# ryanelandt/PressureFieldContact.jl

Hardware: AMD Instinct MI355X
Metric: tet-tri clip+integrate ops/s (higher is better)
Workload: dtype f64

## Files before the change

pressurefieldcontact.jl_amd/csrc/pfc_hip.hip:

```cpp
#include "pfc_kernels.h"

#include <atomic>
#include <condition_variable>
#include <functional>
#include <mutex>
#include <thread>
#include <cmath>
#include <cstdlib>
#include <limits>
#include <cstdarg>
#include <cstdio>
#include <cstring>
#include <string>
#include <vector>

#include "../../include/pfc.h"
#include "pfc_sort.h"

namespace pfc {

__global__ void k_prep_tri(int n, const double *__restrict__ pt, const int *__restrict__ tri, TriRec *__restrict__ out) {
    int k = blockIdx.x * blockDim.x + threadIdx.x;
    if (k >= n) return;
    V3 a = ld3(pt + 3 * tri[3 * k]), b = ld3(pt + 3 * tri[3 * k + 1]), c = ld3(pt + 3 * tri[3 * k + 2]);
// ... 324 lines not shown
    bool want_surv = false;
    int opt_graph = 1;
    size_t fcap = 0, ccap = 0, tcap = 0, rcap = 0;
    DevBuf<double> h_pose;
    int last_n_items = 0, last_levels = 0, last_bfs_levels = 0;
    bool pending = false;
    hipStream_t last_stream = nullptr;
    long long stats[8] = {0, 0, 0, 0, 0, 0, 0, 0};
    DevBuf<double> dual_in, dual_acc, dual_res, dual_out, dual_poly;
    DevBuf<int2> dual_pkey;
    DevBuf<int> dual_sel, dual_flag;
    DevBuf<double> scat_d;
    DevBuf<int> scat_i;
    DevBuf<double> sdual_d, sdual_w;
    DevBuf<int> sdual_i;
    DevBuf<char> sdual_tmp;
    DevBuf<int> surv;
    DevBuf<int> rgn;
    DevBuf<int> poly_item, pcnt, poly_cand;
    DevBuf<double> poly;
    long long last_undecided = 0;
    long long last_active = 0;
    struct ShapeHint { int n = 0; bool sparse = false; } hints[4];
    void note_shape(int n, bool sparse) {
        int k = 0;
        while (k < 3 && hints[k].n != n) ++k;
        for (; k > 0; --k) hints[k] = hints[k - 1];
        hints[0].n = n; hints[0].sparse = sparse;
    }
    bool shape_is_sparse(int n) const {
        for (const ShapeHint &e : hints) if (e.n == n) return e.sparse;
        return false;
    }
    long long last_tslots = 0;
    Event ev[EV_COUNT];
    bool ev_valid = false;
    pfc_context *twin = nullptr;
    bool is_twin = false;
    DevBuf<int> fout;
    PinBuf<int> h_fout;
    int *fout_dev = nullptr;
    const int *fout_host = nullptr;
    int opt_fused = 1;
    int opt_fixed_order = 0;
    DevBuf<int> det;
    DevBuf<unsigned long long> sort_keys[2];
    DevBuf<int> canon_off, canon_fill, canon_item;
    int sort_tmp_items = 0;
    bool fixed_whole_list = false;
    DevBuf<char> sort_tmp;
    size_t sort_tmp_for = 0;
    int sort_tmp_bits = 0;
    int max_elem1 = 1, max_elem2 = 1;
    DevBuf<double> fx_rec, vfx_rec;
    DevBuf<int> vfx_head;
    DevBuf<int> fx_head;
    long long surv_sorted_serial = -1;
    size_t sort_cover = 0;
    size_t sort_cover_used = 0;
    int opt_vertex_fields = 1;
    int opt_clip_queue = 1;
    int fused_skip = 0;
    int fused_seq = 0;
    int fu_nw = 1;
    int last_fu_nw = 0, last_team = 0;
    int n_cu = 0;
    int opt_team = 48;
    DevBuf<unsigned long long> team;
    DevBuf<int> emit_ctr;
    PinBuf<int> h_emit;
    PinBuf<unsigned> h_more;
    bool fu_emit = false;
    int dual_fused_skip = 0;
    const double *fu_dpose = nullptr, *fu_dtwist = nullptr;
    double *fu_dwrench = nullptr, *fu_dsdot = nullptr;
    int fu_ndir = 0;
    bool pending_fused = false, last_fused = false;
    int opt_split_min = 1025;
    int opt_clip_min = 384;
    int opt_poison = 0;
    int split_n0 = 0;
    bool in_split = false;
    int last_parts = 1;
    Event ev_fork, ev_join, ev_join0;
    int twin_queue_fallback = 0;
    DevBuf<long long> surf_cnt, surf_off, surf_out;
    DevBuf<double> surf_part;
    DevBuf<int> surf_seg, surf_canon_off, surf_canon_fill, surf_canon_item;
    DevBuf<double> ljac_seed;
    DevBuf<double> ljac_out;
    DevBuf<double> ljac_io;
    DevBuf<int> ljac_ids;
    std::vector<int> ins_bodies;
    DevBuf<int> bodies_bind;
    bool bodies_stale = true;
    DevBuf<double> bodies_d;
    DevBuf<int> bodies_i;
    DevBuf<unsigned long long> surf_keys[2];
    DevBuf<char> surf_tmp;
    PinBuf<long long> h_surf;
    bool pending_surface = false;
    bool surf_whole_list = false;
    bool surf_cap_short = false;
    int surf_n_ctr = 0;
    long long surf_cap_poly = 0, surf_cap_trac = 0;
    DevBuf<long long> surf_hl;
// ... 230 lines not shown

int record_eval(pfc_context *h, int n_items, const int *d_ins_ids, const double *d_pose, const double *d_twist,
                const double *d_s, double *d_wrench, double *d_sdot, int *d_counts, hipStream_t st, bool prof) {
    new_value_pass(h);
    h->pending_more = false; h->last_dual_reused = false;
    const int levels = eff_levels(h);
    int *ccount = h->ctr.p, *tcount = h->ctr.p + 1, *next_seed = h->ctr.p + 2;
    int *ucount = h->ctr.p + 4, *fcount = h->ctr.p + 6;
    int *pcount = h->ctr.p + ((levels + 9) & ~1);
#ifdef PFC_STAMPS
    HIP_TRY(h, hipMemsetAsync(h->stamps.p, 0, sizeof(unsigned long long) * 16, st));
#endif
    if (prof) HIP_TRY(h, hipEventRecord(h->ev[EV_START], st));

    EvalArgs ea;
    ea.n_items = n_items; ea.ins_ids = d_ins_ids; ea.pose = d_pose; ea.twist = d_twist; ea.s = d_s;
    ea.bp_pose = h->bp_dev;
    ea.ins = h->d_ins; ea.meshes = h->d_meshes; ea.n_ins = (int)h->ins.size(); ea.items = h->items.p;
    ea.frontier0 = h->frontier[0].p; ea.fcount = fcount; ea.acc = h->acc.p; ea.icnt = h->icnt.p;
    ea.status = h->status.p;
    hipLaunchKernelGGL(k_setup_items, dim3(grid_for(n_items, 64, 1 << 20)), dim3(64), 0, st, ea);
    if (prof) HIP_TRY(h, hipEventRecord(h->ev[EV_SETUP], st));

    const int L = bfs_levels_for(h, n_items, levels);
    launch_broadphase(h, n_items, L, ccount, fcount, next_seed, ucount, st);
    if (h->bp_dev)
        hipLaunchKernelGGL(k_repose, dim3(grid_for(n_items, 64, 1 << 20)), dim3(64), 0, st, n_items, d_pose, h->items.p);
    if (h->opt_fixed_order) {
        int ba, bb;
        const int bits = pfc_sort_key_bits(n_items, h->max_elem1, h->max_elem2, &ba, &bb);
        if (bits > 64)
            return fail(h, PFC_ERR_BAD_ARG, "option fixed_order: (item, element, element) needs %d key bits for %d items, more than 64", bits, n_items);
        size_t cover = h->sort_cover ? h->sort_cover : h->ccap;
        if (cover > h->ccap) cover = h->ccap;
        h->sort_cover_used = cover;
        static const bool global_sort = std::getenv("PFC_FIXED_GLOBAL_SORT") != nullptr;
        if (global_sort || h->fixed_whole_list)
            HIP_TRY(h, pfc_sort_candidates(h->cand.p, ccount, cover, h->sort_keys[0].p, h->sort_keys[1].p, h->sort_tmp.p, h->sort_tmp.cap,
                                           n_items, ba, bb, bits, h->status.p, kStFixedCover, st));
        else
            HIP_TRY(h, pfc_canon_candidates(h->cand.p, ccount, cover, h->icnt.p, n_items, h->sort_keys[0].p, h->sort_keys[1].p, h->canon_off.p,
                                            h->canon_fill.p, h->canon_item.p, bb, h->status.p, kStFixedCover, kStFixedBig, st));
        hipLaunchKernelGGL(k_fixed_init, dim3(grid_for(n_items, 256, 1 << 20)), dim3(256), 0, st, n_items, h->det.p);
    }
    if (prof) HIP_TRY(h, hipEventRecord(h->ev[EV_BP], st));

    NpArgs np;
    np.items = h->items.p; np.cand = h->cand.p; np.ccount = ccount; np.ccap = (int)h->ccap; np.acc = h->acc.p;
    np.icnt = h->icnt.p; np.n_items = n_items; np.clip_n = h->opt_debug ? h->clip_n.p : nullptr; np.trac = trac_view(h);
    np.tcount = tcount; np.tcap = (int)h->tcap; np.status = h->status.p; np.debug = h->opt_debug;
    np.stamps = h->stamps.p;
    np.rec = h->rec.p; np.rgn = h->rgn.p; np.rr_cap = (int)(h->rcap / kRgn);
    np.poly_item = h->poly_item.p; np.poly = h->poly.p; np.pcap = (int)poly_cap(h->ccap);
    np.pcnt = h->pcnt.p; np.chunk_switch = kNpChunkSwitch; np.poly_cand = h->want_surv ? h->poly_cand.p : nullptr;
    np.surv = h->want_surv ? h->surv.p : nullptr; np.scount = pcount + 1;
    const int np_grid = grid_for(h->ccap, kNpBlock, kNpMaxBlocks);
    const int np_mode = h->opt_debug ? 1 : ((h->opt_fixed_order || (h->opt_clip_min > 0 && n_items >= h->opt_clip_min)) ? 2 : 0);
    if (np_mode == 1) {
        if (h->any_tet_tet) hipLaunchKernelGGL((k_narrow<true, 1>), dim3(np_grid), dim3(kNpBlock), 0, st, np);
        else hipLaunchKernelGGL((k_narrow<false, 1>), dim3(np_grid), dim3(kNpBlock), 0, st, np);
    } else if (np_mode == 0) {
        if (h->any_tet_tet) hipLaunchKernelGGL((k_narrow<true, 0>), dim3(np_grid), dim3(kNpBlock), 0, st, np);
        else hipLaunchKernelGGL((k_narrow<false, 0>), dim3(np_grid), dim3(kNpBlock), 0, st, np);
    } else {
        if (h->opt_clip_queue && !h->any_tet_tet) {
            hipLaunchKernelGGL(k_clip_queue, dim3(np_grid), dim3(kNpBlock), 0, st, np);
        } else if (h->in_split || (n_items >= 640 && n_items < 1024)) {
            if (h->any_tet_tet) hipLaunchKernelGGL((k_narrow<true, 3>), dim3(np_grid), dim3(kNpBlock), 0, st, np);
            else hipLaunchKernelGGL((k_narrow<false, 3>), dim3(np_grid), dim3(kNpBlock), 0, st, np);
        } else {
            if (h->any_tet_tet) hipLaunchKernelGGL((k_narrow<true, 2>), dim3(np_grid), dim3(kNpBlock), 0, st, np);
            else hipLaunchKernelGGL((k_narrow<false, 2>), dim3(np_grid), dim3(kNpBlock), 0, st, np);
        }
        IntegArgs ig;
        ig.items = h->items.p; ig.n_items = n_items; ig.ccount = ccount; ig.ccap = (int)h->ccap; ig.chunk_switch = kNpChunkSwitch;
        ig.pcnt = h->pcnt.p; ig.poly_item = h->poly_item.p; ig.poly = h->poly.p; ig.pcap = np.pcap;
        ig.poly_cand = np.poly_cand; ig.surv = np.surv; ig.scount = np.scount; ig.acc = h->acc.p; ig.rec = h->rec.p;
        ig.rgn = h->rgn.p; ig.rr_cap = np.rr_cap; ig.icnt = h->icnt.p; ig.status = h->status.p;
        ig.det = h->opt_fixed_order ? h->det.p : nullptr;
        if (h->opt_fixed_order) hipLaunchKernelGGL(k_integ_fixed, dim3(grid_for(h->ccap, 64, kNpMaxBlocks)), dim3(64), 0, st, ig);
        else hipLaunchKernelGGL(k_integ, dim3(grid_for(h->ccap, 64, kNpMaxBlocks)), dim3(64), 0, st, ig);
    }
    if (prof) HIP_TRY(h, hipEventRecord(h->ev[EV_NP], st));

    BrArgs br;
    br.items = h->items.p; br.n_items = n_items; br.acc = h->acc.p; br.res = h->res.p; br.icnt = h->icnt.p;
    br.trac = trac_view(h); br.tcount = tcount; br.tcap = (int)h->tcap; br.wrench = d_wrench; br.sdot = d_sdot;
    br.counts = d_counts;
    br.ctr = h->ctr.p; br.n_ctr = levels + 12; br.status = h->status.p; br.tail = h->tail_dev ? h->tail_dev : h->tail.p;
    br.rgn = h->rgn.p; br.i_pcount = (levels + 9) & ~1;
    if (h->opt_fixed_order && np_mode == 2) {
        FixedArgs fx;
        fx.rec = h->rec.p; fx.det = h->det.p; fx.n_items = n_items; fx.n_slots = (int)(h->rcap / kRgn) * kRgn; fx.items = h->items.p;
        fx.acc = h->acc.p; fx.status = h->status.p;
        hipLaunchKernelGGL(k_shift_fixed, dim3(n_items), dim3(64), 0, st, fx);
    }
    if (h->any_bristle) {
        ShiftArgs sh;
        sh.rec = h->rec.p; sh.rgn = h->rgn.p; sh.rr_cap = (int)(h->rcap / kRgn); sh.acc = h->acc.p;
        if (!(h->opt_fixed_order && np_mode == 2)) hipLaunchKernelGGL(k_shift, dim3(grid_for(h->rcap, 64, 2048)), dim3(64), 0, st, sh);
        hipLaunchKernelGGL(k_eig, dim3(n_items), dim3(64), 0, st, br);
        FricArgs fr;
        fr.items = h->items.p; fr.poly_item = h->poly_item.p; fr.poly = h->poly.p; fr.ccount = ccount; fr.ccap = (int)h->ccap;
        fr.chunk_switch = kNpChunkSwitch; fr.pcnt = h->pcnt.p;
        fr.pcap = np.pcap; fr.res = h->res.p; fr.acc = h->acc.p;
        fr.n_items = n_items; fr.status = h->status.p;
// ... 740 lines not shown
    }
    h->finalized = true;
    return PFC_OK;
}

static int check_eval_args(pfc_context *h, int n_items, const void *ins_ids, const void *pose, const void *twist,
                           const void *s, const void *wrench, const void *sdot) {
    if (!h->finalized) return fail(h, PFC_ERR_STATE, "pfc_eval before pfc_finalize");
    if (n_items < 0) return fail(h, PFC_ERR_BAD_ARG, "negative n_items");
    if (n_items == 0) return PFC_OK;
    if (h->ins.empty()) return fail(h, PFC_ERR_STATE, "no contact instructions");
    if (!pose || !twist || !wrench || !sdot) return fail(h, PFC_ERR_BAD_ARG, "null buffer");
    if (!ins_ids && n_items > (int)h->ins.size())
        return fail(h, PFC_ERR_BAD_ARG, "n_items exceeds the number of instructions and no ins_ids given");
    if (h->any_bristle && !s) return fail(h, PFC_ERR_BAD_ARG, "bristle instructions need the state buffer s");
    return PFC_OK;
}

int pfc_eval_device(pfc_handle h, int n_items, const int *d_ins_ids, const double *d_pose, const double *d_twist,
                    const double *d_s, double *d_wrench, double *d_sdot, int *d_counts, void *stream) {
    if (!h) return PFC_ERR_BAD_ARG;
    if (h->multi)
        return multi_eval_device(h, n_items, 0, d_ins_ids, d_pose, nullptr, d_twist, d_s, nullptr, nullptr, nullptr, d_wrench, d_sdot,
                                 nullptr, nullptr, d_counts, stream);
    { const int rc = check_eval_args(h, n_items, d_ins_ids, d_pose, d_twist, d_s, d_wrench, d_sdot); if (rc != PFC_OK) return rc; }
    if (n_items == 0) { h->pending = false; h->last_n_items = 0; return PFC_OK; }
    HIP_TRY(h, hipSetDevice(h->device));
    hipStream_t st = stream ? (hipStream_t)stream : h->stream;
    h->split_n0 = 0;
    h->pending_fused = false;
    end_kept_pass(h);
    h->pending_more = false;
    int team = fused_team(h, n_items);
    if (team > 1 && !team_acquire(h)) team = fused_ok(h, n_items) ? 1 : 0;
    if (team) {
        h->fu_nw = team;
        const int rc_t = enqueue_fused(h, n_items, d_ins_ids, d_pose, d_twist, d_s, d_wrench, d_sdot, d_counts, st);
        h->fu_nw = 1;
        if (rc_t != PFC_OK) team_release(h);
        return rc_t;
    }
    if (h->fused_skip > 0 && n_items <= kFusedMaxItems) --h->fused_skip;
    const bool split = h->opt_split_min > 0 && n_items >= h->opt_split_min && d_ins_ids && !h->opt_debug && !h->opt_fixed_order &&
                       !h->want_surv && !h->is_twin && !pile_mode(h, n_items);
    if (!split) return enqueue_eval(h, n_items, d_ins_ids, d_pose, d_twist, d_s, d_wrench, d_sdot, d_counts, st);
    int rc = make_twin(h);
    if (rc != PFC_OK) return rc;
    pfc_context *t = h->twin;
    t->opt_profile = h->opt_profile; t->opt_max_levels = h->opt_max_levels; t->opt_bfs_levels = h->opt_bfs_levels;
    t->opt_poison = h->opt_poison;
    if (t->opt_clip_min != h->opt_clip_min) { t->opt_clip_min = h->opt_clip_min; t->ghave[0] = t->ghave[1] = false; }
    if (t->opt_clip_queue != h->opt_clip_queue) { t->opt_clip_queue = h->opt_clip_queue; t->ghave[0] = t->ghave[1] = false; }
    if (t->opt_vertex_fields != h->opt_vertex_fields) { t->opt_vertex_fields = h->opt_vertex_fields; t->ghave[0] = t->ghave[1] = false; }
    t->opt_graph = h->opt_graph;
    if (t->opt_no_filter != h->opt_no_filter) { t->opt_no_filter = h->opt_no_filter; t->ghave[0] = t->ghave[1] = false; }
    const int n0 = n_items / 2, n1 = n_items - n0;
    hipStream_t s0 = h->stream;
    HIP_TRY(h, hipEventRecord(h->ev_fork, st));
    if (s0 != st) HIP_TRY(h, hipStreamWaitEvent(s0, h->ev_fork, 0));
    HIP_TRY(h, hipStreamWaitEvent(t->stream, h->ev_fork, 0));
    h->in_split = true; t->in_split = true;
    rc = enqueue_eval(h, n0, d_ins_ids, d_pose, d_twist, d_s, d_wrench, d_sdot, d_counts, s0);
    h->in_split = false;
    if (rc != PFC_OK) return rc;
    rc = enqueue_eval(t, n1, d_ins_ids + n0, d_pose + 24 * (size_t)n0, d_twist + 6 * (size_t)n0,
                      d_s ? d_s + 6 * (size_t)n0 : nullptr, d_wrench + 6 * (size_t)n0, d_sdot + 6 * (size_t)n0,
                      d_counts ? d_counts + 4 * (size_t)n0 : nullptr, t->stream);
    if (rc != PFC_OK) { h->err = t->err; return rc; }
    HIP_TRY(h, hipEventRecord(h->ev_join, t->stream));
    HIP_TRY(h, hipStreamWaitEvent(st, h->ev_join, 0));
    if (s0 != st) {
        HIP_TRY(h, hipEventRecord(h->ev_join0, s0));
        HIP_TRY(h, hipStreamWaitEvent(st, h->ev_join0, 0));
    }
    h->split_n0 = n0;
    return PFC_OK;
}

namespace {

struct SurfFricOut {
    const double *s;
    double *fric, *fric_summary, *stiff;
};

int surface_enqueue(pfc_context *h, int n_items, const int *d_ins_ids, const double *d_pose, const double *d_twist, long long cap_poly,
                    long long cap_trac, long long *d_poly_off, int *d_poly_idx, double *d_poly_xyz, long long *d_poly_trac,
                    double *d_trac, double *d_summary, int *d_counts, long long *d_totals, hipStream_t st, const SurfFricOut *fo = nullptr) {
    new_value_pass(h);
    h->pending_more = false;
    h->pin_in_pt = {}; h->pin_din_pt = {};
    h->pending = false; h->pending_dual = false; h->pending_dual_hyb = false; h->split_n0 = 0;
    if (h->pending_fused) { h->pending_fused = false; team_release(h); }
    int ba, bb;
    const int bits = pfc_sort_key_bits(n_items, h->max_elem1, h->max_elem2, &ba, &bb);
    if (bits > 64)
        return fail(h, PFC_ERR_BAD_ARG, "pfc_contact_surface: (item, element, element) needs %d key bits for %d items, more than 64", bits, n_items);
    HIP_TRY(h, ensure_work(h, n_items));
    const size_t c = h->ccap;
    HIP_TRY(h, h->surf_cnt.ensure(2 * (c + 1)));
    HIP_TRY(h, h->surf_off.ensure(2 * (c + 1)));
    HIP_TRY(h, h->surf_part.ensure(c * kSurfSums));
    HIP_TRY(h, h->surf_seg.ensure((size_t)n_items + 1));
    HIP_TRY(h, h->surf_canon_off.ensure((size_t)n_items + 1));
    HIP_TRY(h, h->surf_canon_fill.ensure((size_t)n_items));
    HIP_TRY(h, h->surf_canon_item.ensure(c));
// ... 1315 lines not shown
    }
    h->want_surv = true;
    int rc = pfc_eval(h, n_items, ins_ids, pose, twist, s, wrench, sdot, counts);
    h->want_surv = false;
    if (rc != PFC_OK) return rc;
    HIP_TRY(h, ensure_graphed(h, h->dual_in, nk * 36));
    HIP_TRY(h, ensure_graphed(h, h->dual_acc, nk * kDaStride));
    HIP_TRY(h, ensure_graphed(h, h->dual_res, nk * kDrStride));
    HIP_TRY(h, ensure_graphed(h, h->dual_out, nk * 12));
    double *dp = h->dual_in.p, *dt = dp + nk * 24, *dsd = dt + nk * 6;
    const size_t in_bytes = sizeof(double) * nk * 36, out_bytes = sizeof(double) * nk * 12;
    HIP_TRY(h, h->pin_in.ensure(in_bytes));
    HIP_TRY(h, h->pin_out.ensure(out_bytes));
    pack_seeds((double *)h->pin_in.p, nk, d_pose, d_twist, d_s, true);
    HIP_TRY(h, hipMemcpyAsync(dp, h->pin_in.p, in_bytes, hipMemcpyHostToDevice, st));
    rc = launch_dual(h, n_items, n_dir, h->tail.p, dp, dt, dsd, h->dual_out.p, h->dual_out.p + nk * 6, (size_t)h->stats[2], st, nullptr);
    if (rc != PFC_OK) return rc;
    h->dual_hint = h->stats[2];
    HIP_TRY(h, hipMemcpyAsync(h->pin_out.p, h->dual_out.p, out_bytes, hipMemcpyDeviceToHost, st));
    HIP_TRY(h, hipStreamSynchronize(st));
    copy_out_dual((const double *)h->pin_out.p, nk, d_wrench, d_sdot);
    return PFC_OK;
}

int pfc_set_option(pfc_handle h, const char *name, long long value) {
    if (!h || !name) return PFC_ERR_BAD_ARG;
    if (h->multi) {
        if (!std::strcmp(name, "multi_min")) { h->multi->opt_min_items = value < 1 ? 1 : (int)value; h->multi->part_n = 0; return PFC_OK; }
        h->multi->dev_kept = false;
        for (pfc_context *c : h->multi->shard) {
            const int rc = on_shard(h, c, [&](pfc_context *c1) { return pfc_set_option(c1, name, value); });
            if (rc != PFC_OK) return rc;
        }
        return PFC_OK;
    }
    end_kept_pass(h);
    if (!std::strcmp(name, "debug")) h->opt_debug = value != 0;
    else if (!std::strcmp(name, "profile")) h->opt_profile = value != 0;
    else if (!std::strcmp(name, "max_levels")) {
        if (value < 0 || value > (1 << 20) || (h->finalized && value > h->max_levels))
            return fail(h, PFC_ERR_BAD_ARG, "max_levels must be 0 (automatic) or 1..%d (depth of the finalized trees + 1)", h->max_levels);
        h->opt_max_levels = (int)value; h->ghave[0] = h->ghave[1] = false; h->dghave = false;
    }
    else if (!std::strcmp(name, "bfs_levels")) h->opt_bfs_levels = (int)value;
    else if (!std::strcmp(name, "graph")) h->opt_graph = value != 0;
    else if (!std::strcmp(name, "split_min")) h->opt_split_min = (int)value;
    else if (!std::strcmp(name, "dual_reuse")) h->opt_dual_reuse = (int)value;
    else if (!std::strcmp(name, "clip_min")) { h->opt_clip_min = (int)value; h->ghave[0] = h->ghave[1] = false; h->dghave = false; }
    else if (!std::strcmp(name, "clip_queue")) { h->opt_clip_queue = (int)value; h->ghave[0] = h->ghave[1] = false; h->dghave = false; }
    else if (!std::strcmp(name, "vertex_fields")) {
        if (value != 0 && value != 1) return fail(h, PFC_ERR_BAD_ARG, "vertex_fields must be 0 (per-point k_fric) or 1 (per-corner fields)");
        h->opt_vertex_fields = (int)value; h->ghave[0] = h->ghave[1] = false; h->dghave = false;
    }
    else if (!std::strcmp(name, "poison")) h->opt_poison = value != 0;
    else if (!std::strcmp(name, "fused")) { h->opt_fused = value != 0; h->fused_skip = 0; }
    else if (!std::strcmp(name, "team")) h->opt_team = value < 0 ? 0 : (value > kTeamMaxWg ? kTeamMaxWg : (int)value);
    else if (!std::strcmp(name, "team_fault")) h->opt_team_fault = (int)value;
    else if (!std::strcmp(name, "fused_f32")) h->opt_fused_f32 = value != 0;
    else if (!std::strcmp(name, "dual_fold")) { h->opt_dual_fold = value != 0; h->dghave = false; }
    else if (!std::strcmp(name, "fixed_order")) {
        const int on = value != 0;
        if (on != h->opt_fixed_order) {
            h->opt_fixed_order = on; h->fused_skip = 0;
            h->ghave[0] = h->ghave[1] = false; h->dghave = false;
            h->rec.release();
        }
    }
    else if (!std::strcmp(name, "no_filter")) { h->opt_no_filter = (int)value; h->ghave[0] = h->ghave[1] = false; h->dghave = false; }
    else return fail(h, PFC_ERR_BAD_ARG, "unknown option %s", name);
    return PFC_OK;
}

int pfc_get_stats(pfc_handle h, long long *out8) {
    if (!h || !out8) return PFC_ERR_BAD_ARG;
    if (h->multi) { for (int k = 0; k < 8; ++k) out8[k] = h->multi->stats[k]; return PFC_OK; }
    for (int k = 0; k < 8; ++k) out8[k] = h->stats[k];
    return PFC_OK;
}

int pfc_get_stage_ms(pfc_handle h, float *out6) {
    if (!h || !out6) return PFC_ERR_BAD_ARG;
    if (h->multi)
        return on_first_shard(h, [&](pfc_context *c) { return pfc_get_stage_ms(c, out6); });
    if (!h->ev_valid) return fail(h, PFC_ERR_STATE, "profile option was off for the last evaluation");
    HIP_TRY(h, hipSetDevice(h->device));
    HIP_TRY(h, hipEventSynchronize(h->ev[EV_FIN]));
    for (int k = 0; k < 5; ++k) HIP_TRY(h, hipEventElapsedTime(&out6[k], h->ev[k], h->ev[k + 1]));
    HIP_TRY(h, hipEventElapsedTime(&out6[5], h->ev[EV_START], h->ev[EV_FIN]));
    if (h->last_parts == 2 && h->twin && h->twin->ev_valid) {
        pfc_context *t = h->twin;
        float b[6];
        HIP_TRY(h, hipEventSynchronize(t->ev[EV_FIN]));
        for (int k = 0; k < 5; ++k) HIP_TRY(h, hipEventElapsedTime(&b[k], t->ev[k], t->ev[k + 1]));
        HIP_TRY(h, hipEventElapsedTime(&b[5], t->ev[EV_START], t->ev[EV_FIN]));
        for (int k = 0; k < 5; ++k) out6[k] = 0.5f * (out6[k] + b[k]);
        if (b[5] > out6[5]) out6[5] = b[5];
    }
    return PFC_OK;
}

int pfc_last_parts(pfc_handle h) { return h ? (h->multi ? pfc_last_parts(h->multi->shard[0]) : (h->last_fused ? 0 : h->last_parts)) : 0; }
int pfc_last_team(pfc_handle h) { return h ? (h->multi ? pfc_last_team(h->multi->shard[0]) : (h->last_fused ? h->last_fu_nw : 0)) : 0; }
int pfc_last_dual_reused(pfc_handle h) {
    if (!h) return 0;
    if (h->multi) {
        for (int k = 0; k < h->multi->n_used; ++k)
// ... 330 lines not shown
```

pressurefieldcontact.jl_amd/csrc/pfc_np.h:

```cpp
#pragma once

struct TracSoA {
    int *item;
    double *nx, *ny, *nz, *rx, *ry, *rz, *dA, *p;
};

struct NpArgs {
    const ItemRec *items;
    const WorkRec *cand;
    const int *ccount;
    int ccap;
    double *acc;
    double *rec;
    int *rgn;
    int rr_cap;
    int *pcnt;
    int chunk_switch;
    int *poly_cand;
    int *icnt;
    int n_items;
    int *clip_n;
    int *poly_item;
    double *poly;
    int pcap;
    int *surv;
    int *scount;
    TracSoA trac;
    int *tcount;
    int tcap;
    unsigned *status;
    int debug;
    unsigned long long *stamps;
};

__device__ __forceinline__ V3 cross_fma(V3 a, V3 b) {
    return V3{__builtin_fma(a.y, b.z, -(a.z * b.y)), __builtin_fma(a.z, b.x, -(a.x * b.z)), __builtin_fma(a.x, b.y, -(a.y * b.x))};
}
__device__ __forceinline__ double dot_fma(V3 a, V3 b) { return __builtin_fma(a.z, b.z, __builtin_fma(a.y, b.y, a.x * b.x)); }
__device__ __forceinline__ V3 axpy_fma(double a, V3 x, V3 y) {
    return V3{__builtin_fma(a, x.x, y.x), __builtin_fma(a, x.y, y.y), __builtin_fma(a, x.z, y.z)};
}

#ifndef PFC_EXP
#define PFC_EXP 0
#endif
constexpr int kElim = PFC_EXP;
constexpr int kNpBlock = 64;
constexpr int kNpChunkBig = 512;
__device__ __forceinline__ int np_chunk(int n_c, int chunk_switch) {
    int C = kNpChunkBig;
    while (C > kNpBlock && (long long)C * chunk_switch > n_c) C >>= 1;
    return C;
}

constexpr int kRingColsClip = 48;
#define PR(k, c) poly[((((rbase) + (k)) & 7) * 4 + (c)) * RC + rcol]

__device__ __forceinline__ double readlane_f64(double v, int src) {
    return __hiloint2double(__builtin_amdgcn_readlane(__double2hiint(v), src),
                            __builtin_amdgcn_readlane(__double2loint(v), src));
}

__device__ __forceinline__ double wave_total(double v, int lane) {
    double t;
    t = dpp_move<0x111, 0xF>(v); v += t;
    t = dpp_move<0x112, 0xF>(v); v += t;
    t = dpp_move<0x114, 0xF>(v); v += t;
    t = dpp_move<0x118, 0xF>(v); v += t;
    t = dpp_move<0x142, 0xA>(v); v += (lane & 16) ? t : 0.0;
    t = dpp_move<0x143, 0xC>(v); v += (lane >= 32) ? t : 0.0;
// ... 657 lines not shown
                const int n_run = __popcll(heads);
                if (lane < n_run && !((rec_done >> lane) & 1ull) && rbase + lane < g.rr_cap)
                    g.rec[(size_t)(rslot0 + rbase + lane) * kRecStride + 1] = 0.0;
            }
            STAMP(r3);
#ifdef PFC_STAMPS
            st_r[0] += r1 - t4; st_r[1] += r2 - r1; st_r[2] += r3 - r2;
#endif
            if (single) {
                const int n_ne = __popcll(__ballot(has_poly));
                const int ntl = contributed ? n_trac_lane : 0;
                int nt = 0;
#pragma unroll
                for (int b = 0; b < 5; ++b) nt += __popcll(__ballot((ntl >> b) & 1)) << b;
                if (lane == 0 && am) {
                    if (n_ne) atomicAdd(&g.icnt[4 * (size_t)item_first + 2], n_ne);
                    if (nt) atomicAdd(&g.icnt[4 * (size_t)item_first + 3], nt);
                }
            } else {
                count_per_item(g.icnt, cw.item, 2, active, has_poly);
                count_per_item(g.icnt, cw.item, 3, active, contributed, n_trac_lane);
            }
        }
#ifdef PFC_STAMPS
        STAMP(t5);
        {
            if (t1 == 0) t1 = t2;
            st_c[0] += t1 - t0; st_c[1] += t2 - t1; st_c[2] += t3 - t2; st_c[3] += t4 - t3; st_c[4] += t5 - t4; st_c[5] += 1;
        }
#endif
    }
    if (lane == 0) g.pcnt[ch] = pc;
    }
#ifdef PFC_STAMPS
    if (lane == 0 && g.stamps && st_c[5])
    {
        for (int k = 0; k < 6; ++k) atomicAdd(&g.stamps[k], st_c[k]);
        atomicAdd(&g.stamps[6], st_r[0]); atomicAdd(&g.stamps[7], st_r[1]); atomicAdd(&g.stamps[14], st_r[2]);
    }
#endif
}
#undef PR

__global__ void __launch_bounds__(kNpBlock) k_clip_queue(NpArgs g) {
    constexpr int RC = kNpBlock;
    __shared__ double poly[8 * 4 * RC];
    __shared__ unsigned short qpos[2 * kNpBlock];
    const int lane = threadIdx.x;
    int n_c = *g.ccount;
    if (n_c > g.ccap) n_c = g.ccap;
    const int C = np_chunk(n_c, g.chunk_switch);
    const int n_chunk = (n_c + C - 1) / C;
    const unsigned long long below = (1ull << lane) - 1ull;
#define QZ(e, k, i) poly[(((((e) >> 6) * 3 + (k)) * 4 + (i)) * RC) + ((e) & 63)]
#define QX(e, i) poly[(((6 + ((e) >> 6)) * 4 + (i)) * RC) + ((e) & 63)]
    for (int ch = blockIdx.x; ch < n_chunk; ch += gridDim.x) {
        const int n_here = n_c - ch * C < C ? n_c - ch * C : C;
        const int n_round = (n_here + kNpBlock - 1) / kNpBlock;
        int q = 0;
        int pc = 0;
        auto dense_round = [&]() {
            const int n_take = q < kNpBlock ? q : kNpBlock;
            const bool mine = lane < n_take, left = kNpBlock + lane < q;
            V3 nh = mk3(0.0, 0.0, 0.0);
            unsigned long long meta = 0ull;
            int pos = 0;
            if (mine) {
                nh = mk3(QX(lane, 0), QX(lane, 1), QX(lane, 2));
                meta = (unsigned long long)__double_as_longlong(QX(lane, 3));
                pos = (int)qpos[lane];
            }
            double zl[3][4], xl[4];
            int posl = 0;
            if (left) {
#pragma unroll
                for (int k = 0; k < 3; ++k)
#pragma unroll
                    for (int i = 0; i < 4; ++i) zl[k][i] = QZ(kNpBlock + lane, k, i);
#pragma unroll
                for (int i = 0; i < 4; ++i) xl[i] = QX(kNpBlock + lane, i);
                posl = (int)qpos[kNpBlock + lane];
            }
            const int item = (int)(unsigned)(meta & 0xFFFFFFFFull), b = (int)(unsigned)(meta >> 32);
            const ItemRec *it = g.items + item;
            const GTetRec *tp = (const GTetRec *)(it->tet + b);
            RingCol<RC> ring{poly, lane, 0};
            int n_poly = 0;
            double V[12] = {0.0, 0.0, 0.0, 0.0, 0.0, 0.0, 0.0, 0.0, 0.0, 0.0, 0.0, 0.0}, E[4] = {0.0, 0.0, 0.0, 0.0};
            if (mine) {
#pragma unroll
                for (int k = 0; k < 12; ++k) V[k] = tp->xrz[k];
#pragma unroll
                for (int k = 0; k < 4; ++k) E[k] = tp->epsr[k];
            }
            if (mine) {
                bool err = false;
                n_poly = clip_ring_in_tet_coordinates(ring, 3, err);
                if (err) atomicOr(g.status, kStNonFinite);
            }
            const bool has_poly = n_poly >= 3;
            const unsigned long long km = __ballot(has_poly);
            const int slot = ch * C + pc + __popcll(km & below);
            pc += __popcll(km);
            if (has_poly) np_keep_polygon(ring, n_poly, V, E, nh, g, slot, item, ch * C + pos);
            if (km) {
                const int item_first = __builtin_amdgcn_readfirstlane(item);
                if (__all(!mine || item == item_first)) {
                    if (lane == 0) atomicAdd(&g.icnt[4 * (size_t)item_first + 2], __popcll(km));
                } else {
                    count_per_item(g.icnt, item, 2, mine, has_poly);
                }
            }
            if (left) {
#pragma unroll
                for (int k = 0; k < 3; ++k)
#pragma unroll
                    for (int i = 0; i < 4; ++i) QZ(lane, k, i) = zl[k][i];
#pragma unroll
                for (int i = 0; i < 4; ++i) QX(lane, i) = xl[i];
                qpos[lane] = (unsigned short)posl;
            }
            q -= n_take;
            wave_lds_sync();
        };
        for (int rd = 0; rd < n_round; ++rd) {
            const int pos = rd * kNpBlock + lane, idx = ch * C + pos;
            bool active = pos < n_here;
            WorkRec cw;
            cw.item = 0; cw.a = 0; cw.b = 0; cw.pad = 0;
            if (active) cw = g.cand[idx];
            if ((unsigned)cw.item >= (unsigned)g.n_items) {
                atomicOr(g.status, kStHole);
                cw.item = 0; cw.a = 0; cw.b = 0;
                active = false;
            }
            const ItemRec *it = g.items + cw.item;
            const GTetRec *tp = (const GTetRec *)(it->tet + cw.b);
            double z[4][4];
            int n_in = 0;
            V3 nh_in = mk3(0.0, 0.0, 0.0);
            bool survivor = false;
            if (active) survivor = np_front<false>(it, cw, tp, z, n_in, nh_in, g.status, true);
            const unsigned long long sm = __ballot(survivor);
            if (survivor) {
                const int e = q + __popcll(sm & below);
#pragma unroll
                for (int k = 0; k < 3; ++k)
#pragma unroll
                    for (int i = 0; i < 4; ++i) QZ(e, k, i) = z[k][i];
                QX(e, 0) = nh_in.x; QX(e, 1) = nh_in.y; QX(e, 2) = nh_in.z;
                QX(e, 3) = __longlong_as_double((long long)(((unsigned long long)(unsigned)cw.b << 32) | (unsigned long long)(unsigned)cw.item));
                qpos[e] = (unsigned short)pos;
            }
            q += __popcll(sm);
            wave_lds_sync();
            if (q >= kNpBlock) dense_round();
        }
        if (q > 0) dense_round();
        if (lane == 0) g.pcnt[ch] = pc;
    }
#undef QZ
#undef QX
}

struct IntegArgs {
    const ItemRec *items;
    int n_items;
    const int *ccount;
    int ccap, chunk_switch;
    const int *pcnt;
    int *poly_item;
    const double *poly;
    int pcap;
    const int *poly_cand;
    int *surv, *scount;
    double *acc, *rec;
    int *rgn;
    int rr_cap;
    int *icnt;
    unsigned *status;
    int *det;
};

template <int N, int L>
__device__ __forceinline__ double lds_rows_total(const double *buf, int lane, int lane0) {
    constexpr int RS = 64 + L;
    static_assert(N * L <= 64 && (L == 1 || L == 2 || L == 4), "rows x lanes per row must fit the wave");
    double t = 0.0;
    const int row = lane / L, part = lane % L;
    if (row < N) {
        const double *r = buf + row * RS + part;
        double t0 = 0.0, t1 = 0.0, t2 = 0.0, t3 = 0.0;
#pragma unroll
        for (int j = 0; j < 64 / L; j += 8) {
            const double a0 = r[L * j], a1 = r[L * (j + 1)], a2 = r[L * (j + 2)], a3 = r[L * (j + 3)];
            const double a4 = r[L * (j + 4)], a5 = r[L * (j + 5)], a6 = r[L * (j + 6)], a7 = r[L * (j + 7)];
            t0 += a0; t1 += a1; t2 += a2; t3 += a3;
            t0 += a4; t1 += a5; t2 += a6; t3 += a7;
        }
        t = (t0 + t1) + (t2 + t3);
    }
#pragma unroll
    for (int m = 1; m < L; m <<= 1) t += __shfl_xor(t, m, 64);
    const int dst_row = lane - lane0;
    const double out = __shfl(t, (dst_row >= 0 && dst_row < N) ? dst_row * L : 0, 64);
    return (dst_row >= 0 && dst_row < N) ? out : 0.0;
}

template <bool DET>
__device__ __forceinline__ void integ_body(const IntegArgs &g, double *m27) {
    constexpr int RS = 66;
    const int lane = threadIdx.x;
    int n_c = *g.ccount;
    if (n_c > g.ccap) n_c = g.ccap;
    const int C = np_chunk(n_c, g.chunk_switch);
    const int n_chunk = (n_c + C - 1) / C;
    const size_t P = (size_t)g.pcap;
    for (int ch = blockIdx.x; ch < n_chunk; ch += gridDim.x) {
        int cnt = __builtin_amdgcn_readfirstlane(g.pcnt[ch]);
        if (cnt > C) cnt = C;
        int cur = -1, n_tr = 0;
        bool cur_reg = false;
        V3 c0 = mk3(0.0, 0.0, 0.0);
        double s10[10];
#pragma unroll
        for (int k = 0; k < 10; ++k) s10[k] = 0.0;
        auto flush = [&]() {
            if (cur < 0 || !__any(n_tr > 0)) return;
            double t10 = 0.0, Wt = 0.0, sx = 0.0, sy = 0.0, sz = 0.0;
#pragma unroll
            for (int k = 0; k < 10; ++k) {
                const double t = wave_total(s10[k], lane);
                if (lane == (DET ? kRecTen + k : k)) t10 = t;
                if (k == 6) Wt = t;
                if (k == 7) sx = t;
                if (k == 8) sy = t;
                if (k == 9) sz = t;
            }
            if constexpr (DET) {
                const bool mom = !cur_reg && Wt > 0.0;
                double mine = 0.0;
                if (mom) {
                    wave_lds_sync();
                    mine = lds_rows_total<27, 2>(m27, lane, 5);
                    if (lane == 1) mine = Wt;
                    if (lane == 2) mine = c0.x;
                    if (lane == 3) mine = c0.y;
                    if (lane == 4) mine = c0.z;
                    if (lane == 32) mine = sx - Wt * c0.x;
                    if (lane == 33) mine = sy - Wt * c0.y;
                    if (lane == 34) mine = sz - Wt * c0.z;
                }
                if (lane == 0) mine = (double)cur;
                if (lane >= kRecTen && lane < kRecTen + 10) mine = t10;
                if (lane == kRecChunk) mine = (double)ch;
                const int rgn_c = ch & (kRgn - 1);
                int rs = 0;
                if (lane == 0) rs = atomicAdd(g.rgn + rgn_c * kRgnStride + 1, 1);
                rs = __builtin_amdgcn_readfirstlane(rs);
                if (rs < g.rr_cap) {
                    const int slot = rgn_c * g.rr_cap + rs;
                    if (lane == kRecNext) mine = (double)atomicExch(&g.det[3 * (size_t)cur], slot);
                    if (lane == kRecNext + 1) { atomicMin(&g.det[3 * (size_t)cur + 1], ch); atomicMax(&g.det[3 * (size_t)cur + 2], ch); }
                    if (lane < kRecStrideFixed) g.rec[(size_t)slot * kRecStrideFixed + lane] = mine;
                } else if (lane == 0) {
                    atomicOr(g.status, kStRecOvf);
                }
                if (mom) wave_lds_sync();
            } else {
            if (lane < 10 && t10 != 0.0) unsafeAtomicAdd(&g.acc[(size_t)cur * kAccStride + lane], t10);
            if (!cur_reg && Wt > 0.0) {
                wave_lds_sync();
                double mine = lds_rows_total<27, 2>(m27, lane, 5);
                if (lane == 0) mine = (double)cur;
                if (lane == 1) mine = Wt;
                if (lane == 2) mine = c0.x;
                if (lane == 3) mine = c0.y;
                if (lane == 4) mine = c0.z;
                if (lane == 32) mine = sx - Wt * c0.x;
                if (lane == 33) mine = sy - Wt * c0.y;
                if (lane == 34) mine = sz - Wt * c0.z;
                const int rgn_c = ch & (kRgn - 1);
                int rs = 0;
                if (lane == 0) rs = atomicAdd(g.rgn + rgn_c * kRgnStride + 1, 1);
                rs = __builtin_amdgcn_readfirstlane(rs);
                if (rs < g.rr_cap) {
                    if (lane < kRecStride) g.rec[((size_t)rgn_c * g.rr_cap + rs) * kRecStride + lane] = mine;
                } else if (lane == 0) {
                    atomicOr(g.status, kStRecOvf);
                }
                wave_lds_sync();
            }
            }
            const int nt = wave_total_i(n_tr, lane);
            if (lane == 0 && nt) atomicAdd(&g.icnt[4 * (size_t)cur + 3], nt);
        };
        for (int p0 = 0; p0 < cnt; p0 += 64) {
            const int idx = ch * C + p0 + lane;
            const bool active = p0 + lane < cnt;
            unsigned pk = active ? (unsigned)g.poly_item[idx] : 0u;
            if ((pk >> 28) > 8u || ((pk >> 28) >= 3u && (pk & 0x0FFFFFFFu) >= (unsigned)g.n_items)) {
                atomicOr(g.status, kStHole);
                pk = 0u;
            }
            const int n = (int)(pk >> 28);
            const bool has = n >= 3;
            const int item = has ? (int)(pk & 0x0FFFFFFFu) : -1;
            const double *o = g.poly + idx;
            V3 nh = mk3(0.0, 0.0, 0.0), cen = nh;
            double er0 = 0.0, er1 = 0.0, er2 = 0.0, er3 = 0.0;
            if (has) {
                nh = mk3(o[0], o[P], o[2 * P]);
                cen = mk3(o[3 * P], o[4 * P], o[5 * P]);
                er0 = o[6 * P]; er1 = o[7 * P]; er2 = o[8 * P]; er3 = o[9 * P];
            }
            const ItemRec *it = g.items + (has ? item : 0);
            const bool lane_reg = it->model == PFC_REGULARIZED;
            const int nq = it->nq;
            const V3 w = ld3(it->w), vl = ld3(it->v);
            const double chi = it->chi, Ebar = it->Ebar;
            int ntl = 0;
            double W = 0.0, wr1[3] = {0.0, 0.0, 0.0}, wrr[6] = {0.0, 0.0, 0.0, 0.0, 0.0, 0.0};
            double fs[6] = {0.0, 0.0, 0.0, 0.0, 0.0, 0.0};
            if (has) {
                V3 v2 = mk3(o[(10 + 3 * (n - 1)) * P], o[(11 + 3 * (n - 1)) * P], o[(12 + 3 * (n - 1)) * P]);
                V3 vn = mk3(o[10 * P], o[11 * P], o[12 * P]);
                PointParams pp;
                pp.w = w; pp.vl = vl; pp.chi = chi; pp.Ebar = Ebar; pp.er0 = er0; pp.er1 = er1; pp.er2 = er2; pp.er3 = er3; pp.nq = nq;
                auto points = [&](auto &&body) {
                    for (int k = 0; k < n; ++k) {
                        const V3 v1 = v2;
                        v2 = vn;
                        if (k + 1 < n) vn = mk3(o[(13 + 3 * k) * P], o[(14 + 3 * k) * P], o[(15 + 3 * k) * P]);
                        ntl += fan_triangle_points(pp, v1, v2, cen, nh, body);
                    }
                };
                if (lane_reg) {
                    const double v_c = it->v_c, mu_s = it->mu_s, mu_d = it->mu_d;
                    points([&](const V3 &r, const V3 &rdot, double p, double dA) {
                        const double p_dA = p * dA;
                        const V3 vt = vec_sub_vec_proj(rdot, nh);
                        const double m2 = dot_fma(vt, vt);
                        V3 T;
                        if (m2 < v_c * v_c) {
                            T = vt * (-(mu_s / v_c));
                        } else {
                            double ri = __builtin_amdgcn_rsq(m2);
                            const double hm = 0.5 * m2;
                            ri = ri * __builtin_fma(-hm * ri, ri, 1.5);
                            ri = ri * __builtin_fma(-hm * ri, ri, 1.5);
                            const double mg = m2 * ri;
                            const double mu = clamped_piecewise(mg, 2 * v_c, 3 * v_c, mu_s, mu_d);
// ... 37 lines not shown
#pragma unroll
                        for (int k = 0; k < 27; ++k) m27[k * RS + lane] = 0.0;
                    }
                }
                if (!in_run || !contributed) continue;
                n_tr += ntl;
                if (reg) {
#pragma unroll
                    for (int k = 0; k < 6; ++k) s10[k] += fs[k];
                } else {
                    const V3 Sr = mk3(wr1[0] + W * cen.x, wr1[1] + W * cen.y, wr1[2] + W * cen.z);
                    const V3 ta = cross(Sr, nh);
                    s10[0] += ta.x; s10[1] += ta.y; s10[2] += ta.z;
                    s10[3] += nh.x * W; s10[4] += nh.y * W; s10[5] += nh.z * W;
                    s10[6] += W; s10[7] += Sr.x; s10[8] += Sr.y; s10[9] += Sr.z;
                    const V3 d = cen - c0;
                    const V3 m1 = mk3(wr1[0] + W * d.x, wr1[1] + W * d.y, wr1[2] + W * d.z);
                    double q[6];
                    q[0] = wrr[0] + 2.0 * wr1[0] * d.x + W * d.x * d.x;
                    q[1] = wrr[1] + wr1[0] * d.y + wr1[1] * d.x + W * d.x * d.y;
                    q[2] = wrr[2] + wr1[0] * d.z + wr1[2] * d.x + W * d.x * d.z;
                    q[3] = wrr[3] + 2.0 * wr1[1] * d.y + W * d.y * d.y;
                    q[4] = wrr[4] + wr1[1] * d.z + wr1[2] * d.y + W * d.y * d.z;
                    q[5] = wrr[5] + 2.0 * wr1[2] * d.z + W * d.z * d.z;
                    double *mc = m27 + lane;
#define M27_(k, v) mc[(k) * RS] += (v)
                    M27_(0, W * nh.x * nh.x); M27_(1, W * nh.x * nh.y); M27_(2, W * nh.x * nh.z);
                    M27_(3, W * nh.y * nh.y); M27_(4, W * nh.y * nh.z); M27_(5, W * nh.z * nh.z);
                    const V3 an = cross(m1, nh);
                    M27_(6, an.x * nh.x); M27_(7, an.y * nh.x); M27_(8, an.z * nh.x);
                    M27_(9, an.x * nh.y); M27_(10, an.y * nh.y); M27_(11, an.z * nh.y);
                    M27_(12, an.x * nh.z); M27_(13, an.y * nh.z); M27_(14, an.z * nh.z);
                    const V3 q0c = mk3(q[0], q[1], q[2]), q1c = mk3(q[1], q[3], q[4]), q2c = mk3(q[2], q[4], q[5]);
                    const V3 m0 = cross(nh, q0c), m1c = cross(nh, q1c), m2c = cross(nh, q2c);
                    const V3 r0 = cross(nh, mk3(m0.x, m1c.x, m2c.x)), r1 = cross(nh, mk3(m0.y, m1c.y, m2c.y));
                    const V3 r2 = cross(nh, mk3(m0.z, m1c.z, m2c.z));
                    M27_(15, r0.x); M27_(16, r0.y); M27_(17, r0.z); M27_(18, r1.y); M27_(19, r1.z); M27_(20, r2.z);
#pragma unroll
                    for (int k = 0; k < 6; ++k) M27_(21 + k, q[k]);
#undef M27_
                }
            }
            if (has && (!contributed || lane_reg)) g.poly_item[idx] = 0;
            if (g.surv != nullptr) {
                const unsigned long long sm = __ballot(has);
                if (sm) {
                    int sbase = 0;
                    if (lane == 0) sbase = atomicAdd(g.scount, __popcll(sm));
                    sbase = __builtin_amdgcn_readfirstlane(sbase);
                    if (has) g.surv[sbase + __popcll(sm & ((1ull << lane) - 1ull))] = contributed ? g.poly_cand[idx] : -1;
                }
            }
        }
        flush();
    }
}
__global__ void __launch_bounds__(64, 2) k_integ(IntegArgs g) {
    __shared__ double m27[27 * 66];
    integ_body<false>(g, m27);
}
__global__ void __launch_bounds__(64, 2) k_integ_fixed(IntegArgs g) {
    __shared__ double m27[27 * 66];
    integ_body<true>(g, m27);
}

struct FricArgs {
    const ItemRec *items;
    const int *poly_item;
    const double *poly;
    const int *ccount;
    int ccap, chunk_switch;
    const int *pcnt;
    int pcap;
    int n_items;
    unsigned *status;
    const double *res;
    double *acc;
    FixedSink sink;
};
template <bool FX, bool VF>
__device__ __forceinline__ void fric_body(const FricArgs &g) {
    const int lane = threadIdx.x;
    const size_t P = (size_t)g.pcap;
    int n_c = *g.ccount;
    if (n_c > g.ccap) n_c = g.ccap;
    const int C = np_chunk(n_c, g.chunk_switch);
    const int n_chunk = (n_c + C - 1) / C;
    for (int ch = blockIdx.x; ch < n_chunk; ch += gridDim.x) {
      int cnt = __builtin_amdgcn_readfirstlane(g.pcnt[ch]);
      if (cnt > C) cnt = C;
      for (int p0 = 0; p0 < cnt; p0 += 64) {
        const int idx = ch * C + p0 + lane;
        const bool active = p0 + lane < cnt;
        double sum[6];
#pragma unroll
        for (int k = 0; k < 6; ++k) sum[k] = 0.0;
        int item = 0;
        bool contributed = false;
        unsigned pk = active ? (unsigned)g.poly_item[idx] : 0u;
        if ((pk >> 28) > 8u || ((pk >> 28) >= 3u && (pk & 0x0FFFFFFFu) >= (unsigned)g.n_items)) {
            atomicOr(g.status, kStHole);
            pk = 0u;
        }
        if ((pk >> 28) >= 3u) {
            item = (int)(pk & 0x0FFFFFFFu);
            const int n = (int)(pk >> 28);
            const ItemRec *it = g.items + item;
            const double *o = g.poly + idx;
            const V3 nh = mk3(o[0], o[P], o[2 * P]);
            const V3 cen = mk3(o[3 * P], o[4 * P], o[5 * P]);
            const double er0 = o[6 * P], er1 = o[7 * P], er2 = o[8 * P], er3 = o[9 * P];
            const int nq = it->nq;
            const V3 w = ld3(it->w), vl = ld3(it->v);
            const double chi = it->chi, Ebar = it->Ebar, mu_s = it->mu_s, mu_d = it->mu_d;
            const double tau = it->tau, k_bar = it->k_bar;
            const double mu_slope = (mu_d - mu_s) / (3 * mu_s - 2 * mu_s);
            const double *res = g.res + (size_t)item * kResStride;
            const V3 cop = ld3(res + kResCop), Da = ld3(res + kResDelta), Dl = ld3(res + kResDelta + 3);
            const V3 ts_c0 = ((Dl - cross(Da, cop)) + vl * tau) * (-k_bar), ts_e = (Da + w * tau) * (-k_bar);
            V3 v2 = mk3(o[(10 + 3 * (n - 1)) * P], o[(11 + 3 * (n - 1)) * P], o[(12 + 3 * (n - 1)) * P]);
            V3 vn = mk3(o[10 * P], o[11 * P], o[12 * P]);
            PointParams pp;
            pp.w = w; pp.vl = vl; pp.chi = chi; pp.Ebar = Ebar; pp.er0 = er0; pp.er1 = er1; pp.er2 = er2; pp.er3 = er3; pp.nq = nq;
            if constexpr (VF) {
                const FanFields ff = fan_fields(pp);
                const double mu_s2 = mu_s * mu_s;
                const double a_c = fan_field_a(ff, cen), d_c = fan_field_d(ff, cen);
                const V3 Ts_c0 = ts_c0 + cross_fma(ts_e, cen);
                const V3 ts_c = axpy_fma(-dot_fma(Ts_c0, nh), nh, Ts_c0);
                const V3 x_c = cen - cop;
                struct Corner { V3 c, r; double a, d; V3 ts; };
                auto corner = [&](const V3 &c) {
                    Corner f;
                    f.c = c; f.r = c - cen;
                    f.a = fan_linear_a(ff, f.r); f.d = fan_linear_d(ff, f.r);
                    const V3 Ts = cross_fma(ts_e, f.r);
                    f.ts = axpy_fma(-dot_fma(Ts, nh), nh, Ts);
                    return f;
                };
                Corner f2 = corner(v2);
                for (int k = 0; k < n; ++k) {
                    const Corner f1 = f2;
                    f2 = corner(vn);
                    if (k + 1 < n) vn = mk3(o[(13 + 3 * k) * P], o[(14 + 3 * k) * P], o[(15 + 3 * k) * P]);
                    const double area = triangle_area(f1.c, f2.c, cen, nh);
                    if (!(0.0 < area)) continue;
// ... 10 lines not shown
                            double ri = __builtin_amdgcn_rsq(m2);
                            const double hm = 0.5 * m2;
                            ri = ri * __builtin_fma(-hm * ri, ri, 1.5);
                            ri = ri * __builtin_fma(-hm * ri, ri, 1.5);
                            const double mg = m2 * ri;
                            const double y = mu_s + (mg - 2 * mu_s) * mu_slope;
                            const double mu = (y > mu_s) ? mu_s : ((y < mu_d) ? mu_d : y);
                            sc *= mu * ri;
                        }
                        const V3 xt = cross_fma(x, Ts);
                        sum[0] = __builtin_fma(sc, xt.x, sum[0]); sum[1] = __builtin_fma(sc, xt.y, sum[1]);
                        sum[2] = __builtin_fma(sc, xt.z, sum[2]); sum[3] = __builtin_fma(sc, Ts.x, sum[3]);
                        sum[4] = __builtin_fma(sc, Ts.y, sum[4]); sum[5] = __builtin_fma(sc, Ts.z, sum[5]);
                    };
                    auto at = [&](const Corner &q) { point(fan_at(ff, Sa, q.a), fan_at(ff, Sd, q.d), fan_at(ff, Sts, q.ts), fan_at(ff, Sx, q.r)); };
                    at(f2);
                    if (ff.nq != 1) { at(f1); point(Sa, Sd, Sts, Sx); }
                }
            } else {
            for (int k = 0; k < n; ++k) {
                const V3 v1 = v2;
                v2 = vn;
                if (k + 1 < n) vn = mk3(o[(13 + 3 * k) * P], o[(14 + 3 * k) * P], o[(15 + 3 * k) * P]);
                if (fan_triangle_points(pp, v1, v2, cen, nh, [&](const V3 &r, const V3 &, double p, double dA) {
                    const double p_dA = p * dA;
                    const V3 x = r - cop;
                    V3 Ts = ts_c0 + cross_fma(ts_e, r);
                    Ts = axpy_fma(-dot_fma(Ts, nh), nh, Ts);
                    const double m2 = dot_fma(Ts, Ts);
                    V3 T;
                    if (m2 < mu_s * mu_s) {
                        T = Ts;
                    } else {
                        double ri = __builtin_amdgcn_rsq(m2);
                        const double hm = 0.5 * m2;
                        ri = ri * __builtin_fma(-hm * ri, ri, 1.5);
                        ri = ri * __builtin_fma(-hm * ri, ri, 1.5);
                        const double mg = m2 * ri;
                        const double y = mu_s + (mg - 2 * mu_s) * mu_slope;
                        const double mu = (y > mu_s) ? mu_s : ((y < mu_d) ? mu_d : y);
                        T = Ts * (mu * ri);
                    }
                    const V3 Tc = T * p_dA;
                    const V3 ta = cross_fma(x, Tc);
                    sum[0] += ta.x; sum[1] += ta.y; sum[2] += ta.z;
                    sum[3] += Tc.x; sum[4] += Tc.y; sum[5] += Tc.z;
                }))
                    contributed = true;
            }
            }
        }
        accumulate_items<6, FX>(g.acc, item, FX ? (active && (pk >> 28) >= 3u) : active, contributed, sum, kAccFric, kAccStride, &g.sink, (ch * C + p0) >> 6);
      }
    }
}
template <bool VF> __global__ void __launch_bounds__(64, 3) k_fric(FricArgs g) { fric_body<false, VF>(g); }
template <bool VF> __global__ void __launch_bounds__(64, 3) k_fric_fixed(FricArgs g) { fric_body<true, VF>(g); }
```

Measured before the change: 4.106 billion.

## Partition clipped polygons by vertex count into front/back chunk segments

After: 4.146 billion, median of 6. Within noise of the previous version (+1.0%).

```diff
diff --git a/pressurefieldcontact.jl_amd/csrc/pfc_hip.hip b/pressurefieldcontact.jl_amd/csrc/pfc_hip.hip
--- a/pressurefieldcontact.jl_amd/csrc/pfc_hip.hip
+++ b/pressurefieldcontact.jl_amd/csrc/pfc_hip.hip
@@ -400,6 +400,7 @@
     size_t sort_tmp_for = 0;
     int sort_tmp_bits = 0;
     int max_elem1 = 1, max_elem2 = 1;
+    int opt_poly_split = 4;
     DevBuf<double> fx_rec, vfx_rec;
     DevBuf<int> vfx_head;
     DevBuf<int> fx_head;
@@ -736,6 +737,7 @@
     np.stamps = h->stamps.p;
     np.rec = h->rec.p; np.rgn = h->rgn.p; np.rr_cap = (int)(h->rcap / kRgn);
     np.poly_item = h->poly_item.p; np.poly = h->poly.p; np.pcap = (int)poly_cap(h->ccap);
+    np.split_n = (h->opt_fixed_order || h->opt_debug) ? 0 : h->opt_poly_split;
     np.pcnt = h->pcnt.p; np.chunk_switch = kNpChunkSwitch; np.poly_cand = h->want_surv ? h->poly_cand.p : nullptr;
     np.surv = h->want_surv ? h->surv.p : nullptr; np.scount = pcount + 1;
     const int np_grid = grid_for(h->ccap, kNpBlock, kNpMaxBlocks);
@@ -1582,6 +1584,7 @@
     if (t->opt_clip_min != h->opt_clip_min) { t->opt_clip_min = h->opt_clip_min; t->ghave[0] = t->ghave[1] = false; }
     if (t->opt_clip_queue != h->opt_clip_queue) { t->opt_clip_queue = h->opt_clip_queue; t->ghave[0] = t->ghave[1] = false; }
     if (t->opt_vertex_fields != h->opt_vertex_fields) { t->opt_vertex_fields = h->opt_vertex_fields; t->ghave[0] = t->ghave[1] = false; }
+    if (t->opt_poly_split != h->opt_poly_split) { t->opt_poly_split = h->opt_poly_split; t->ghave[0] = t->ghave[1] = false; }
     t->opt_graph = h->opt_graph;
     if (t->opt_no_filter != h->opt_no_filter) { t->opt_no_filter = h->opt_no_filter; t->ghave[0] = t->ghave[1] = false; }
     const int n0 = n_items / 2, n1 = n_items - n0;
@@ -3003,6 +3006,11 @@
         if (value != 0 && value != 1) return fail(h, PFC_ERR_BAD_ARG, "vertex_fields must be 0 (per-point k_fric) or 1 (per-corner fields)");
         h->opt_vertex_fields = (int)value; h->ghave[0] = h->ghave[1] = false; h->dghave = false;
     }
+    else if (!std::strcmp(name, "poly_split")) {
+        if (value != 0 && !((value & ~16LL) >= 3 && (value & ~16LL) <= 7))
+            return fail(h, PFC_ERR_BAD_ARG, "poly_split must be 0 (off), 3..7 (largest vertex count of a chunk's front class, 512-candidate chunks) or that + 16 (every chunk size)");
+        h->opt_poly_split = (int)value; h->ghave[0] = h->ghave[1] = false; h->dghave = false;
+    }
     else if (!std::strcmp(name, "poison")) h->opt_poison = value != 0;
     else if (!std::strcmp(name, "fused")) { h->opt_fused = value != 0; h->fused_skip = 0; }
     else if (!std::strcmp(name, "team")) h->opt_team = value < 0 ? 0 : (value > kTeamMaxWg ? kTeamMaxWg : (int)value);
diff --git a/pressurefieldcontact.jl_amd/csrc/pfc_np.h b/pressurefieldcontact.jl_amd/csrc/pfc_np.h
--- a/pressurefieldcontact.jl_amd/csrc/pfc_np.h
+++ b/pressurefieldcontact.jl_amd/csrc/pfc_np.h
@@ -16,6 +16,7 @@
     int rr_cap;
     int *pcnt;
     int chunk_switch;
+    int split_n;
     int *poly_cand;
     int *icnt;
     int n_items;
@@ -779,13 +780,14 @@
     const int C = np_chunk(n_c, g.chunk_switch);
     const int n_chunk = (n_c + C - 1) / C;
     const unsigned long long below = (1ull << lane) - 1ull;
+    const int split_n = (g.split_n >= 16 || C == kNpChunkBig) ? (g.split_n & 15) : 0;
 #define QZ(e, k, i) poly[(((((e) >> 6) * 3 + (k)) * 4 + (i)) * RC) + ((e) & 63)]
 #define QX(e, i) poly[(((6 + ((e) >> 6)) * 4 + (i)) * RC) + ((e) & 63)]
     for (int ch = blockIdx.x; ch < n_chunk; ch += gridDim.x) {
         const int n_here = n_c - ch * C < C ? n_c - ch * C : C;
         const int n_round = (n_here + kNpBlock - 1) / kNpBlock;
         int q = 0;
-        int pc = 0;
+        int pc = 0, pcb = 0;
         auto dense_round = [&]() {
             const int n_take = q < kNpBlock ? q : kNpBlock;
             const bool mine = lane < n_take, left = kNpBlock + lane < q;
@@ -826,9 +828,11 @@
                 if (err) atomicOr(g.status, kStNonFinite);
             }
             const bool has_poly = n_poly >= 3;
-            const unsigned long long km = __ballot(has_poly);
-            const int slot = ch * C + pc + __popcll(km & below);
-            pc += __popcll(km);
+            const bool at_back = has_poly && split_n > 0 && n_poly > split_n;
+            const unsigned long long km = __ballot(has_poly), kb = __ballot(at_back), kf = km & ~kb;
+            const int slot = ch * C + (at_back ? C - 1 - (pcb + __popcll(kb & below)) : pc + __popcll(kf & below));
+            pc += __popcll(kf);
+            pcb += __popcll(kb);
             if (has_poly) np_keep_polygon(ring, n_poly, V, E, nh, g, slot, item, ch * C + pos);
             if (km) {
                 const int item_first = __builtin_amdgcn_readfirstlane(item);
@@ -884,11 +888,23 @@
             if (q >= kNpBlock) dense_round();
         }
         if (q > 0) dense_round();
-        if (lane == 0) g.pcnt[ch] = pc;
+        if (lane == 0) g.pcnt[ch] = pc | (pcb << 16);
     }
 #undef QZ
 #undef QX
 }
+
+struct ChunkEnds {
+    int front, back;
+    __device__ __forceinline__ ChunkEnds(int packed, int C) {
+        front = packed & 0xFFFF; back = (int)((unsigned)packed >> 16);
+        if (front > C) front = C;
+        if (back > C - front) back = C - front;
+    }
+    __device__ __forceinline__ int lo(int seg, int C) const { return seg ? C - back : 0; }
+    __device__ __forceinline__ int hi(int seg, int C) const { return seg ? C : front; }
+    __device__ __forceinline__ int first_piece(int seg, int C) const { return seg ? (C - back) & ~63 : 0; }
+};
 
 struct IntegArgs {
     const ItemRec *items;
@@ -944,8 +960,7 @@
     const int n_chunk = (n_c + C - 1) / C;
     const size_t P = (size_t)g.pcap;
     for (int ch = blockIdx.x; ch < n_chunk; ch += gridDim.x) {
-        int cnt = __builtin_amdgcn_readfirstlane(g.pcnt[ch]);
-        if (cnt > C) cnt = C;
+        const ChunkEnds ends(__builtin_amdgcn_readfirstlane(g.pcnt[ch]), C);
         int cur = -1, n_tr = 0;
         bool cur_reg = false;
         V3 c0 = mk3(0.0, 0.0, 0.0);
@@ -1022,9 +1037,12 @@
             const int nt = wave_total_i(n_tr, lane);
             if (lane == 0 && nt) atomicAdd(&g.icnt[4 * (size_t)cur + 3], nt);
         };
-        for (int p0 = 0; p0 < cnt; p0 += 64) {
+#pragma unroll 1
+        for (int seg = 0; seg < 2; ++seg) {
+        const int lo = ends.lo(seg, C), hi = ends.hi(seg, C);
+        for (int p0 = ends.first_piece(seg, C); p0 < hi; p0 += 64) {
             const int idx = ch * C + p0 + lane;
-            const bool active = p0 + lane < cnt;
+            const bool active = p0 + lane >= lo && p0 + lane < hi;
             unsigned pk = active ? (unsigned)g.poly_item[idx] : 0u;
             if ((pk >> 28) > 8u || ((pk >> 28) >= 3u && (pk & 0x0FFFFFFFu) >= (unsigned)g.n_items)) {
                 atomicOr(g.status, kStHole);
@@ -1168,6 +1186,7 @@
                 }
             }
         }
+        }
         flush();
     }
 }
@@ -1203,11 +1222,13 @@
     const int C = np_chunk(n_c, g.chunk_switch);
     const int n_chunk = (n_c + C - 1) / C;
     for (int ch = blockIdx.x; ch < n_chunk; ch += gridDim.x) {
-      int cnt = __builtin_amdgcn_readfirstlane(g.pcnt[ch]);
-      if (cnt > C) cnt = C;
-      for (int p0 = 0; p0 < cnt; p0 += 64) {
+      const ChunkEnds ends(__builtin_amdgcn_readfirstlane(g.pcnt[ch]), C);
+#pragma unroll 1
+      for (int seg = 0; seg < 2; ++seg) {
+      const int lo = ends.lo(seg, C), hi = ends.hi(seg, C);
+      for (int p0 = ends.first_piece(seg, C); p0 < hi; p0 += 64) {
         const int idx = ch * C + p0 + lane;
-        const bool active = p0 + lane < cnt;
+        const bool active = p0 + lane >= lo && p0 + lane < hi;
         double sum[6];
 #pragma unroll
         for (int k = 0; k < 6; ++k) sum[k] = 0.0;
@@ -1324,6 +1345,7 @@
         }
         accumulate_items<6, FX>(g.acc, item, FX ? (active && (pk >> 28) >= 3u) : active, contributed, sum, kAccFric, kAccStride, &g.sink, (ch * C + p0) >> 6);
       }
+      }
     }
 }
 template <bool VF> __global__ void __launch_bounds__(64, 3) k_fric(FricArgs g) { fric_body<false, VF>(g); }
```
